# xmed-lab/NEURONS

Measured on AMD Instinct MI355X. Metric: denoising frames/sec, 16f x 256^2 clip, 50 DDIM steps, higher is better.
Workload: dtype bf16; 1 GPU; BASELINE config 2: 1 clip(s) per call, (1,4,16,32,32) latent, 50 DDIM steps, CFG 8.5 (batch 2), SparseCtrl + temporal U-Net per step, random-init weights; clips_per_gpu=5, ddim_steps=50, hip_graph=True, output_finite=True, attention=bf16

## Files before the change

neurons_amd/csrc/gemm_route.h:

```cpp
#pragma once
#include "common.h"
#include <cstdlib>
#include <initializer_list>

inline bool env_not_0(const char* name) {
  const char* v = getenv(name);
  return !(v && v[0] == '0');
}

inline int nr_plan_rows(const NrGemmParams& p) { return (p.plan_m > 0 && p.plan_m < p.M) ? p.plan_m : p.M; }

inline int nr_lds_opt_in(unsigned long long& mask, std::initializer_list<const void*> fns, size_t bytes) {
  int dev = 0;
  (void)hipGetDevice(&dev);
  const unsigned long long bit = 1ull << (dev & 63);
  if (mask & bit) return 0;
  for (const void* fn : fns)
    if (hipFuncSetAttribute(fn, hipFuncAttributeMaxDynamicSharedMemorySize, (int)bytes) != hipSuccess) return 2;
  mask |= bit;
  return 0;
}

enum NrGemmClass { NR_GEMM_SMALLM, NR_GEMM_LIN160, NR_GEMM_ROWPANEL, NR_GEMM_G8P, NR_GEMM_TILED, NR_GEMM_NCLASS };
inline const char* const nr_gemm_class_name[NR_GEMM_NCLASS] = {"smallm", "lin160", "rowpanel", "gemm8p", "tiled"};
enum NrWeightLayout { NR_W_ROWMAJOR, NR_W_TAP_INNER, NR_W_FRAGMAJOR, NR_W_LIN160, NR_W_LIN128Q, NR_W_FRAGMAJOR_E4M3 };

struct TiledPlan { int bm, bn, splitk, stages, waves, adma, lin; };
struct SmallmPlan { int nt, G, J, C; };
struct Lin160Plan { int form, big, J, cgmajor; };
struct RowPanelPlan { int nsplit; };
struct G8pPlan { int nt, phases; };

struct NrGemmRoute {
  int cls;
  int weight_layout;
  int m_fast;
  size_t ws_bytes;
  TiledPlan tiled;
  SmallmPlan smallm;
  Lin160Plan lin160;
  RowPanelPlan rowpanel;
  G8pPlan g8p;
};
```

neurons_amd/csrc/lin160.hip:

```cpp
#include "launchers.h"
#include "device_prims.h"
#include <cstdlib>

namespace {

NR_STAMP_BUF(lin160_stamp_buf, 512, 128);
#define L1_STAMP(slot) NR_STAMP_PUT(lin160_stamp_buf, slot)
#ifdef NR_STAMP_FINE
#define Q_STAMPW(slot) NR_STAMP_PUT_AT((threadIdx.x & 63) == 0 && (wave == 0 || wave == 4) && blockIdx.x < 256, lin160_stamp_buf, blockIdx.x + (wave ? 256 : 0), slot)
#else
#define Q_STAMPW(slot) do { } while (0)
#endif

constexpr int L1_BN = 160, L1_NT = 10;
constexpr int L1_W_STAGE = 24 * 1024;
constexpr int L1_NS = 3;

struct NrLin160Params {
  const bf16* x; int lda;
  const bf16* stream;
  const float* bias;
  const bf16* res; int ldr;
  bf16* out; int ldo;
  int M, N, K;
  const float* ln_c; float ln_eps;
  int norot;
};

template <int BM, int MODE = 0>
__global__ __launch_bounds__(512) void lin160_kernel(NrLin160Params p) {
  constexpr bool GLN = MODE == 1;
  static_assert(!GLN || BM == 128, "the GEGLU variant pairs the (value, gate) tiles inside one wave");
  constexpr int RT = BM / 16;
  constexpr int NTW = BM == 128 ? L1_NT : L1_NT / 2;
  constexpr int A_STAGE = BM * 128;
  constexpr int A_PW = BM == 128 ? 2 : 1;
  constexpr int STAGE = L1_W_STAGE + A_STAGE;
  constexpr int PPW = 3 + A_PW;
  extern __shared__ __attribute__((aligned(16))) unsigned char smem[];

  const int tid = threadIdx.x;
  const int lane = tid & 63;
  const int wave = __builtin_amdgcn_readfirstlane(tid >> 6);
  const int fr = lane & 15, fg = lane >> 4;
  const int rt = BM == 128 ? wave : (wave & 3);
  const int n0 = BM == 128 ? 0 : (wave >> 2) * NTW;

  L1_STAMP(0);
  const int NCB = p.N / L1_BN, S = p.K >> 6;
  const int nrg = p.M / BM;
  int rg, cb;
  if ((nrg & 7) == 0) { const int j = blockIdx.x >> 3; cb = j % NCB; rg = (j / NCB) * 8 + (int)(blockIdx.x & 7); }
  else { cb = (int)(blockIdx.x % NCB); rg = blockIdx.x / NCB; }
  const int r0 = rg * BM;
  const int rot = p.norot ? 0 : rg % S;

  const unsigned lds0 = nr_lds_addr(smem);
  const char* wsrc = reinterpret_cast<const char*>(p.stream) + (size_t)cb * ((size_t)S * L1_W_STAGE) + (size_t)(wave * 3) * 1024 + (size_t)lane * 16;
  const bf16* arow;
  {
    const int r = lane >> 2;
    arow = p.x + (size_t)(r0 + 16 * rt + r) * p.lda + (((lane & 3) ^ ((-(r >> 2)) & 3)) << 3);
  }
  auto issue_piece = [&](int s, int slot, int i) {
    const unsigned dst = lds0 + (unsigned)(slot * STAGE);
    int st = s + rot; if (st >= S) st -= S;
    if (i < 3) nr_glds16(wsrc + (size_t)st * L1_W_STAGE + (size_t)i * 1024, dst + (unsigned)((wave * 3 + i) * 1024));
    else {
      const int kk = BM == 128 ? i - 3 : (wave >> 2);
      nr_glds16(arow + 64 * st + 32 * kk, dst + (unsigned)(L1_W_STAGE + (kk * RT + rt) * 1024));
    }
  };
#pragma unroll
  for (int s = 0; s < L1_NS - 1; ++s)
#pragma unroll
    for (int i = 0; i < PPW; ++i) issue_piece(s, s, i);

  L1_STAMP(1);
  f32x4 acc[NTW];
#pragma unroll
  for (int n = 0; n < NTW; ++n) acc[n] = f32x4{0.f, 0.f, 0.f, 0.f};
  float s1 = 0.f, s2 = 0.f;
  const bf16x2 one2 = {(bf16)1.0f, (bf16)1.0f};
  const unsigned wl = (unsigned)(n0 * 1024 + lane * 16);
  const unsigned al = (unsigned)(L1_W_STAGE + rt * 1024 + fr * 64 + ((fg ^ ((-(fr >> 2)) & 3)) << 4));

  int slot = 0;
  for (int s = 0; s < S; ++s) {
    if (s + 1 < S) nr_wait_vmcnt<(L1_NS - 2) * PPW>(); else nr_wait_vmcnt<0>();
    if (s < 40) L1_STAMP(2 + 3 * s);
    __builtin_amdgcn_s_barrier();
    if (s < 40) L1_STAMP(3 + 3 * s);
    const int s_next = s + L1_NS - 1;
    const bool pf = s_next < S;
    int pslot = slot + L1_NS - 1; if (pslot >= L1_NS) pslot -= L1_NS;
    const unsigned char* base = smem + slot * STAGE;
#pragma unroll
    for (int kk = 0; kk < 2; ++kk) {
      const bf16x8 xa = *(const bf16x8*)(base + al + kk * (RT * 1024));
      if constexpr (GLN) {
#pragma unroll
        for (int e = 0; e < 4; ++e) {
          const bf16x2 pr = {xa[2 * e], xa[2 * e + 1]};
          s1 = __builtin_amdgcn_fdot2_f32_bf16(pr, one2, s1, false);
          s2 = __builtin_amdgcn_fdot2_f32_bf16(pr, pr, s2, false);
        }
      }
      bf16x8 w[NTW];
#pragma unroll
      for (int n = 0; n < NTW; ++n) w[n] = *(const bf16x8*)(base + (unsigned)((kk * L1_NT + n) * 1024) + wl);
      if (pf) {
        if (kk == 0) { issue_piece(s_next, pslot, 0); issue_piece(s_next, pslot, 1); }
        else { issue_piece(s_next, pslot, 2); issue_piece(s_next, pslot, 3); if (A_PW == 2) issue_piece(s_next, pslot, 4); }
      }
      __builtin_amdgcn_sched_barrier(0);
#pragma unroll
      for (int n = 0; n < NTW; ++n) acc[n] = __builtin_amdgcn_mfma_f32_16x16x32_bf16(w[n], xa, acc[n], 0, 0, 0);
      __builtin_amdgcn_sched_barrier(0);
    }
    if (s < 40) L1_STAMP(4 + 3 * s);
    slot = slot + 1 == L1_NS ? 0 : slot + 1;
  }
  L1_STAMP(125);

  if constexpr (GLN) {
    const float inv_k = 1.0f / (float)p.K;
    const float mu = nr_rows_sum(s1) * inv_k;
    const float rstd = rsqrtf(fmaxf(nr_rows_sum(s2) * inv_k - mu * mu, 0.f) + p.ln_eps);
    const int row = r0 + 16 * rt + fr;
    const int nb = cb * L1_BN + 4 * fg;
    bf16* orow = p.out + (size_t)row * p.ldo + cb * (L1_BN / 2) + 4 * fg;
#pragma unroll
    for (int i = 0; i < L1_NT / 2; ++i) {
      const int nv = nb + 32 * i, ng = nv + 16;
      const f32x4 cv = *(const f32x4*)(p.ln_c + nv), cg = *(const f32x4*)(p.ln_c + ng);
      const f32x4 bv = *(const f32x4*)(p.bias + nv), bg = *(const f32x4*)(p.bias + ng);
      bf16x4 o;
#pragma unroll
      for (int e = 0; e < 4; ++e) {
        const float v = (acc[2 * i][e] - mu * cv[e]) * rstd + bv[e];
        const float g = (acc[2 * i + 1][e] - mu * cg[e]) * rstd + bg[e];
        o[e] = (bf16)(v * gelu_erf_fast(g));
      }
      nr_store8(orow + 16 * i, o);
    }
    L1_STAMP(126);
    return;
  }
  const int row = r0 + 16 * rt + fr;
  const int cbase = cb * L1_BN + 16 * n0;
  bf16* orow = p.out + (size_t)row * p.ldo + cbase;
  const bf16* rrow = p.res ? p.res + (size_t)row * p.ldr + cbase : nullptr;
#pragma unroll
  for (int k = 0; k < NTW / 2; ++k) {
    f32x4 lo = acc[2 * k], hi = acc[2 * k + 1];
#pragma unroll
    for (int e = 0; e < 4; ++e) {
      auto sw = __builtin_amdgcn_permlane16_swap(__float_as_uint(lo[e]), __float_as_uint(hi[e]), false, false);
      lo[e] = __uint_as_float(sw[0]); hi[e] = __uint_as_float(sw[1]);
    }
    const int c = 16 * (2 * k + (fg & 1)) + 4 * (fg & 2);
    if (p.bias) { lo += *(const f32x4*)(p.bias + cbase + c); hi += *(const f32x4*)(p.bias + cbase + c + 4); }
    if (rrow) {
      const bf16x8 r = *(const bf16x8*)(rrow + c);
#pragma unroll
      for (int e = 0; e < 4; ++e) { lo[e] += (float)r[e]; hi[e] += (float)r[4 + e]; }
    }
    bf16x8 o;
#pragma unroll
    for (int e = 0; e < 4; ++e) { o[e] = (bf16)lo[e]; o[4 + e] = (bf16)hi[e]; }
    nr_store16(orow + c, o);
  }
  if constexpr (NTW % 2 == 1) {
    constexpr int n = NTW - 1;
    const int c = 16 * n + 4 * fg;
    f32x4 v = acc[n];
    if (p.bias) v += *(const f32x4*)(p.bias + cbase + c);
    if (rrow) {
      const bf16x4 r = *(const bf16x4*)(rrow + c);
#pragma unroll
      for (int e = 0; e < 4; ++e) v[e] += (float)r[e];
    }
    bf16x4 o;
#pragma unroll
    for (int e = 0; e < 4; ++e) o[e] = (bf16)v[e];
    nr_store8(orow + c, o);
  }
  L1_STAMP(126);
}

__global__ __launch_bounds__(256) void lin160_w_pack_kernel(const bf16* __restrict__ w, bf16* __restrict__ stream, int N, int K) {
  const int S = K >> 6, NCB = N / L1_BN, CH_STAGE = L1_W_STAGE / 16;
  const long long idx = (long long)blockIdx.x * 256 + threadIdx.x;
  if (idx >= (long long)NCB * S * CH_STAGE) return;
  const int cb = (int)(idx / ((long long)S * CH_STAGE));
  int c = (int)(idx - (long long)cb * S * CH_STAGE);
  const int st = c / CH_STAGE;
  c -= st * CH_STAGE;
  bf16x8 v = bf16x8_zero();
  if (c < 2 * L1_NT * 64) {
    const int kk = c / (L1_NT * 64), n = (c / 64) % L1_NT, lane = c & 63;
    v = *(const bf16x8*)(w + (size_t)(cb * L1_BN + 16 * n + (lane & 15)) * K + 64 * st + 32 * kk + 8 * (lane >> 4));
  }
  *(bf16x8*)(stream + (size_t)idx * 8) = v;
}


constexpr int Q_BN = 128, Q_NT = 8;
constexpr int Q_STAGE = 32 * 1024;
constexpr int Q_NS = 4;

struct NrLin128QParams {
  const bf16* x; int lda;
  const bf16* stream;
  const float* ln_c; const float* bias; float ln_eps;
  bf16* out; int ldo;
  int M, N, J, NCG;
  int norot;
  int cgmajor;
};

template <int KS, bool GEGLU, bool KSPLIT = false>
__global__ __launch_bounds__(512) void lin128q_kernel(NrLin128QParams p) {
  constexpr int K = 32 * KS;
  constexpr int KSL = KSPLIT ? KS / 2 : KS;
  constexpr int KPS = KSPLIT ? 8 : 4;
  constexpr int S = KS / KPS;
  constexpr int BN = KSPLIT ? 64 : Q_BN, NTB = BN / 16;
  constexpr int NS = KSPLIT ? 3 : Q_NS;
  constexpr int XCH = KSPLIT ? 32 * 1024 : 0;
  static_assert(KSL == 20 && S == 5, "20 k-steps per wave in 5 stages of 4");
  extern __shared__ __attribute__((aligned(16))) unsigned char smem[];
  const int tid = threadIdx.x;
  const int lane = tid & 63;
  const int wave = __builtin_amdgcn_readfirstlane(tid >> 6);
  const int fr = lane & 15, fg = lane >> 4;
  const int rp = wave & 3, ch = wave >> 2;
  L1_STAMP(0);
  const int J = p.J;
  int rg, cg;
  const int nrg = p.M >> 7;
  if (!p.cgmajor && (nrg & 7) == 0) { const int i = blockIdx.x >> 3; cg = i % p.NCG; rg = (i / p.NCG) * 8 + (int)(blockIdx.x & 7); }
  else { cg = (int)(blockIdx.x % p.NCG); rg = (int)(blockIdx.x / p.NCG); }
  const int row0 = rg * 128 + 32 * rp + fr;
  const int rot = p.norot ? 0 : rg % S;
  const int G = J * S;

  const unsigned lds0 = nr_lds_addr(smem);
  const char* wbase = reinterpret_cast<const char*>(p.stream) + (size_t)cg * J * ((size_t)S * Q_STAGE) + (size_t)(wave * 4) * 1024 + (size_t)lane * 16;
  auto issue_piece = [&](int g, int i) {
    const int gs = g < G ? g : G - 1;
    const int j = gs / S;
    int st = gs - j * S + rot; if (st >= S) st -= S;
    nr_glds16(wbase + ((size_t)j * S + st) * Q_STAGE + (size_t)i * 1024, lds0 + (unsigned)((g % NS) * Q_STAGE + (wave * 4 + i) * 1024));
  };
#pragma unroll
  for (int g = 0; g < NS - 1; ++g)
#pragma unroll
    for (int i = 0; i < 4; ++i) issue_piece(g, i);

  L1_STAMP(122);
  float* tab = reinterpret_cast<float*>(smem + NS * Q_STAGE + XCH);
  for (int i = tid; i < J * BN; i += 512) {
    tab[i] = p.ln_c[cg * J * BN + i];
    tab[J * BN + i] = p.bias[cg * J * BN + i];
  }

  L1_STAMP(123);
  bf16x8 xb[2][KSL];
#pragma unroll
  for (int rt = 0; rt < 2; ++rt) {
    const bf16* xr = p.x + (size_t)(row0 + 16 * rt) * p.lda + 8 * fg;
#pragma unroll
    for (int ks = 0; ks < KSL; ++ks) {
      int sq = (ks >> 2) + rot; if (sq >= S) sq -= S;
      const int kq = KPS * sq + (KSPLIT ? 4 * ch : 0) + (ks & 3);
      xb[rt][ks] = *(const bf16x8*)(xr + 32 * kq);
    }
  }
  L1_STAMP(124);
  float mu[2], rstd[2];
  {
    bf16x8 ones;
#pragma unroll
    for (int e = 0; e < 8; ++e) ones[e] = (bf16)1.0f;
    float sx[2], sq2[2];
#pragma unroll
    for (int rt = 0; rt < 2; ++rt) {
      f32x4 a1 = {0.f, 0.f, 0.f, 0.f}, a2 = {0.f, 0.f, 0.f, 0.f};
#pragma unroll
      for (int ks = 0; ks < KSL; ++ks) {
        a1 = __builtin_amdgcn_mfma_f32_16x16x32_bf16(ones, xb[rt][ks], a1, 0, 0, 0);
        a2 = __builtin_amdgcn_mfma_f32_16x16x32_bf16(xb[rt][ks], xb[rt][ks], a2, 0, 0, 0);
      }
      const int e_d = fr & 3;
      float d = e_d == 0 ? a2[0] : e_d == 1 ? a2[1] : e_d == 2 ? a2[2] : a2[3];
      d = (fg == (fr >> 2)) ? d : 0.f;
      sx[rt] = a1[0];
      sq2[rt] = nr_rows_sum(d);
    }
    if constexpr (KSPLIT) {
      float* xs = reinterpret_cast<float*>(smem + NS * Q_STAGE);
      if (fg == 0) {
#pragma unroll
        for (int rt = 0; rt < 2; ++rt) { xs[((wave * 2 + rt) * 2 + 0) * 16 + fr] = sx[rt]; xs[((wave * 2 + rt) * 2 + 1) * 16 + fr] = sq2[rt]; }
      }
      __builtin_amdgcn_s_barrier();
#pragma unroll
      for (int rt = 0; rt < 2; ++rt) { sx[rt] += xs[(((wave ^ 4) * 2 + rt) * 2 + 0) * 16 + fr]; sq2[rt] += xs[(((wave ^ 4) * 2 + rt) * 2 + 1) * 16 + fr]; }
    }
#pragma unroll
    for (int rt = 0; rt < 2; ++rt) {
      mu[rt] = sx[rt] * (1.0f / K);
      rstd[rt] = rsqrtf(fmaxf(sq2[rt] * (1.0f / K) - mu[rt] * mu[rt], 0.f) + p.ln_eps);
    }
  }
  L1_STAMP(127);
  nr_wait_vmcnt<0>();
  __builtin_amdgcn_s_barrier();
  L1_STAMP(1);

  const unsigned wl = (unsigned)((KSPLIT ? 16 * ch : 4 * ch) * 1024 + lane * 16);
  const unsigned oofs = (unsigned)row0 * (unsigned)p.ldo + (unsigned)((KSPLIT ? (GEGLU ? 16 * ch : 32 * ch) : (GEGLU ? 32 * ch : 64 * ch)) + 4 * fg);
  bf16x8 w[4];
#pragma unroll
  for (int n = 0; n < 4; ++n) w[n] = *(const bf16x8*)(smem + (unsigned)(n * 1024) + wl);
  f32x4 acc[2][4];
  auto epilogue = [&](int jb) {
    const int cb = cg * J + jb;
    constexpr int NF = KSPLIT ? 2 : 4;
    const float* tc = tab + jb * BN + 16 * (NF * ch) + 4 * fg;
    const float* tb = tc + J * BN;
    if constexpr (KSPLIT) {
      f32x4* ex = reinterpret_cast<f32x4*>(smem + NS * Q_STAGE);
#pragma unroll
      for (int rt = 0; rt < 2; ++rt)
#pragma unroll
        for (int nn = 0; nn < 2; ++nn) {
          f32x4 theirs;
#pragma unroll
          for (int e = 0; e < 4; ++e) theirs[e] = ch ? acc[rt][nn][e] : acc[rt][2 + nn][e];
          ex[((wave * 2 + rt) * 2 + nn) * 64 + lane] = theirs;
        }
      __builtin_amdgcn_s_barrier();
      const f32x4 c0 = *(const f32x4*)(tc), c1 = *(const f32x4*)(tc + 16), b0 = *(const f32x4*)(tb), b1 = *(const f32x4*)(tb + 16);
#pragma unroll
      for (int rt = 0; rt < 2; ++rt) {
        const f32x4 o0 = ex[(((wave ^ 4) * 2 + rt) * 2 + 0) * 64 + lane], o1 = ex[(((wave ^ 4) * 2 + rt) * 2 + 1) * 64 + lane];
        bf16x4 r0, r1;
#pragma unroll
        for (int e = 0; e < 4; ++e) {
          const float t0 = ((ch ? acc[rt][2][e] : acc[rt][0][e]) + o0[e] - mu[rt] * c0[e]) * rstd[rt] + b0[e];
          const float t1 = ((ch ? acc[rt][3][e] : acc[rt][1][e]) + o1[e] - mu[rt] * c1[e]) * rstd[rt] + b1[e];
          if constexpr (GEGLU) r0[e] = (bf16)(t0 * gelu_erf_fast(t1));
          else { r0[e] = (bf16)t0; r1[e] = (bf16)t1; }
        }
        bf16* orow = p.out + (oofs + (unsigned)(16 * rt) * (unsigned)p.ldo + (unsigned)(cb * (GEGLU ? BN / 2 : BN)));
        nr_store8(orow, r0);
        if constexpr (!GEGLU) nr_store8(orow + 16, r1);
      }
    } else if constexpr (GEGLU) {
#pragma unroll
      for (int i = 0; i < NF / 2; ++i) {
        const f32x4 cv = *(const f32x4*)(tc + 32 * i), cgv = *(const f32x4*)(tc + 32 * i + 16);
        const f32x4 bv = *(const f32x4*)(tb + 32 * i), bg = *(const f32x4*)(tb + 32 * i + 16);
#pragma unroll
        for (int rt = 0; rt < 2; ++rt) {
          bf16x4 o;
#pragma unroll
          for (int e = 0; e < 4; ++e) {
            const float v = (acc[rt][2 * i][e] - mu[rt] * cv[e]) * rstd[rt] + bv[e];
            const float gt = (acc[rt][2 * i + 1][e] - mu[rt] * cgv[e]) * rstd[rt] + bg[e];
            o[e] = (bf16)(v * gelu_erf_fast(gt));
          }
          nr_store8(p.out + (oofs + (unsigned)(16 * rt) * (unsigned)p.ldo + (unsigned)(cb * (BN / 2) + 16 * i)), o);
        }
      }
    } else {
#pragma unroll
      for (int n = 0; n < NF; ++n) {
        const f32x4 c4 = *(const f32x4*)(tc + 16 * n), b4 = *(const f32x4*)(tb + 16 * n);
#pragma unroll
        for (int rt = 0; rt < 2; ++rt) {
          bf16x4 o;
#pragma unroll
          for (int e = 0; e < 4; ++e) o[e] = (bf16)((acc[rt][n][e] - mu[rt] * c4[e]) * rstd[rt] + b4[e]);
          nr_store8(p.out + (oofs + (unsigned)(16 * rt) * (unsigned)p.ldo + (unsigned)(cb * BN + 16 * n)), o);
        }
      }
    }
  };
  const f32x4 zero4 = {0.f, 0.f, 0.f, 0.f};
  int g = 0, slot = 0;
  for (int j = 0; j < J; ++j) {
#pragma unroll
    for (int st = 0; st < S; ++st) {
      const int nslot = slot + 1 == NS ? 0 : slot + 1;
#pragma unroll
      for (int kk = 0; kk < 4; ++kk) {
        const unsigned char* nbase;
        if (kk < 3) nbase = smem + slot * Q_STAGE + (kk + 1) * (NTB * 1024);
        else {
          nr_wait_vmcnt<(NS - 2) * 4>();
          asm volatile("s_waitcnt lgkmcnt(0)" ::: "memory");
          if (g < 40) L1_STAMP(2 + 3 * g);
          __builtin_amdgcn_s_barrier();
          if (g < 40) L1_STAMP(3 + 3 * g);
          nbase = smem + nslot * Q_STAGE;
        }
        __builtin_amdgcn_sched_barrier(0);
        if (kk == 0) {
#pragma unroll
          for (int i = 0; i < 4; ++i) issue_piece(g + NS - 1, i);
        }
        __builtin_amdgcn_sched_barrier(0);
#pragma unroll
        for (int n = 0; n < 4; ++n) {
#pragma unroll
          for (int rt = 0; rt < 2; ++rt)
            acc[rt][n] = __builtin_amdgcn_mfma_f32_16x16x32_bf16(w[n], xb[rt][4 * st + kk], (st == 0 && kk == 0) ? zero4 : acc[rt][n], 0, 0, 0);
          __builtin_amdgcn_sched_barrier(0);
          w[n] = *(const bf16x8*)(nbase + (unsigned)(n * 1024) + wl);
          __builtin_amdgcn_sched_barrier(0);
        }
      }
      if (g < 40) L1_STAMP(4 + 3 * g);
      ++g;
      slot = nslot;
    }
    epilogue(j);
    if constexpr (KSPLIT) {
      __builtin_amdgcn_sched_barrier(0);
#pragma unroll
      for (int n = 0; n < 4; ++n) w[n] = *(const bf16x8*)(smem + slot * Q_STAGE + (unsigned)(n * 1024) + wl);
    }
  }
  L1_STAMP(125);
  nr_wait_vmcnt<0>();
  L1_STAMP(126);
}

__global__ __launch_bounds__(256) void lin128q_w_pack_kernel(const bf16* __restrict__ w, bf16* __restrict__ stream, int N, int K, int BN, int KPS) {
  const int S = K / (32 * KPS), CH_STAGE = Q_STAGE / 16, NTB = BN / 16;
  const long long idx = (long long)blockIdx.x * 256 + threadIdx.x;
  if (idx >= (long long)(N / BN) * S * CH_STAGE) return;
  const int cb = (int)(idx / ((long long)S * CH_STAGE));
  int c = (int)(idx - (long long)cb * S * CH_STAGE);
  const int st = c / CH_STAGE;
  c -= st * CH_STAGE;
  const int kk = c / (NTB * 64), n = (c / 64) % NTB, lane = c & 63;
  *(bf16x8*)(stream + (size_t)idx * 8) = *(const bf16x8*)(w + (size_t)(cb * BN + 16 * n + (lane & 15)) * K + 32 * (KPS * st + kk) + 8 * (lane >> 4));
}

}

#ifdef NR_STAMP
extern "C" int nr_lin160_stamp_read(void* dst, size_t bytes, int clear) { return nr_stamp_read_buf(lin160_stamp_buf, dst, bytes, clear); }
#endif

extern "C" size_t nr_lin160_stream_bytes(int N, int K) { return (N % L1_BN == 0 && K % 64 == 0) ? (size_t)(N / L1_BN) * (K / 64) * L1_W_STAGE : 0; }

extern "C" int nr_lin160_panel_rule(int Mp, int N, int K) {
  static const bool off = !env_not_0("NR_LIN160") || !env_not_0("NR_LIN160_PANEL");
  static const bool off1280 = !env_not_0("NR_LIN160_PANEL_K1280");
  static const int maxm = getenv("NR_LIN160_PANEL_MAXM") ? atoi(getenv("NR_LIN160_PANEL_MAXM")) : (1 << 30);
  if (off || Mp < 2048 || Mp > maxm || N < 3 * K) return 0;
  if (K == 640) return Mp >= 4096 && N % Q_BN == 0;
  if (K == 1280) return !off1280 && N % 64 == 0;
  return 0;
}
extern "C" size_t nr_lin128q_stream_bytes(int N, int K) {
  if (K == 640) return N % Q_BN == 0 ? (size_t)N * K * sizeof(bf16) : 0;
  if (K == 1280) return N % 64 == 0 ? (size_t)N * K * sizeof(bf16) : 0;
  return 0;
}
extern "C" int nr_launch_lin128q_w_pack(const bf16* w, int N, int K, bf16* stream, hipStream_t s) {
  const long long total = (long long)(nr_lin128q_stream_bytes(N, K) / 16);
  if (!total) return 1;
  hipLaunchKernelGGL(lin128q_w_pack_kernel, dim3((unsigned)((total + 255) / 256)), dim3(256), 0, s, w, stream, N, K, K == 1280 ? 64 : Q_BN, K == 1280 ? 8 : 4);
  return 0;
}

extern "C" bool lin160_plan(const NrGemmParams& p, Lin160Plan* pl) {
  static const bool off = !env_not_0("NR_LIN160");
  const int Mp = nr_plan_rows(p);
  *pl = Lin160Plan{0, 0, 0, 0};
  const bool ln_wide = p.ln_c && p.bias && p.ksize == 1 && p.stride == 1 && !p.ups && !p.a1 && !p.c1 && !p.rowvec && !p.act && !p.out_f32 && !p.res &&
                       p.out_scale == 1.0f && p.K == p.c0 && p.M % 128 == 0 && p.lda0 % 8 == 0 && p.ldo % 4 == 0;
  if (ln_wide && nr_lin160_panel_rule(Mp, p.N, p.K) &&
      (long long)p.M * p.ldo < (1ll << 31)) {
    const bool ksplit = p.K == 1280;
    const int bn = ksplit ? 64 : Q_BN, ncq = p.N / bn, S = 5, nrg = p.M / 128, ns = ksplit ? 3 : Q_NS;
    static const int j_force = getenv("NR_LIN160_PANEL_J") ? atoi(getenv("NR_LIN160_PANEL_J")) : 0;
    int J = 0; long long best = 0;
    for (int c = 1; c <= 16 && c <= ncq; ++c) {
      if (ncq % c != 0 || c * S < ns - 1) continue;
      const long long wgs = (long long)nrg * (ncq / c), cost = ((wgs + 255) / 256) * (c * S + 6);
      if (!J || cost <= best) { J = c; best = cost; }
    }
    if (j_force > 0 && ncq % j_force == 0 && j_force <= 16) J = j_force;
    pl->form = 4; pl->J = J;
    if (J) {
      static const int cg_force = getenv("NR_LIN160_PANEL_CGMAJOR") ? atoi(getenv("NR_LIN160_PANEL_CGMAJOR")) : -1;
      const int NCG = ncq / J;
      const double wb = 2.0 * p.N * (double)p.K, xb = 2.0 * p.M * (double)p.K;
      const bool can = NCG % 8 == 0 || 8 % NCG == 0;
      const double by_rg = 8.0 * wb + xb;
      const double by_cg = (NCG % 8 == 0 ? 1.0 : 8.0 / NCG) * wb + (NCG % 8 == 0 ? 8.0 : (double)NCG) * xb;
      pl->cgmajor = (can && by_cg < by_rg) ? 1 : 0;
      if (cg_force >= 0) pl->cgmajor = cg_force && can;
    }
    return true;
  }
  static const bool gln_on = env_not_0("NR_LIN160_GEGLU");
  if (!off && gln_on && ln_wide && p.geglu && p.K == 1280 && p.N % L1_BN == 0 && p.N >= 8192 && Mp <= 1024 && (long long)(Mp / 128) * (p.N / L1_BN) >= 192) {
    pl->form = 2;
    return true;
  }
  if (off || p.ksize != 1 || p.stride != 1 || p.ups || p.a1 || p.c1 || p.geglu || p.ln_c || p.rowvec || p.act || p.out_f32 || p.tap_inner) return false;
  if (p.out_scale != 1.0f || p.K != p.c0 || (p.K != 640 && p.K != 1280) || p.N % L1_BN != 0 || p.N > 1280) return false;
  if (p.M % 64 != 0 || Mp < 2048) return false;
  if (p.lda0 % 8 != 0 || p.ldo % 8 != 0 || (p.res && p.ldr % 8 != 0)) return false;
  if (Mp > 8192) return false;
  pl->form = 1;
  pl->big = p.M % 128 == 0 && (long long)(Mp / 128) * (p.N / L1_BN) >= 256;
  return true;
}

extern "C" int nr_launch_lin160_w_pack(const bf16* w, int N, int K, bf16* stream, hipStream_t s) {
  const long long total = (long long)(nr_lin160_stream_bytes(N, K) / 16);
  if (!total) return 1;
  hipLaunchKernelGGL(lin160_w_pack_kernel, dim3((unsigned)((total + 255) / 256)), dim3(256), 0, s, w, stream, N, K);
  return 0;
}

extern "C" int nr_launch_lin160(const NrGemmParams* pp, const Lin160Plan* pl, const bf16* stream, hipStream_t s) {
  const NrGemmParams& g = *pp;
  if (!stream) return 1;
  if (pl->form == 4) {
    const bool ksplit = g.K == 1280;
    if (!g.ln_c || !g.bias || (g.K != 640 && !ksplit) || g.M % 128 != 0 || (long long)g.M * g.ldo >= (1ll << 31)) return 1;
    const int bn = ksplit ? 64 : Q_BN, ncq = g.N / bn, nrg = g.M / 128, ns = ksplit ? 3 : Q_NS, J = pl->J;
    if (g.N % bn != 0 || J < 1 || J > 16 || ncq % J != 0) return 1;
    NrLin128QParams q;
    q.x = g.a0; q.lda = g.lda0; q.stream = stream; q.ln_c = g.ln_c; q.bias = g.bias; q.ln_eps = g.ln_eps; q.out = g.out; q.ldo = g.ldo; q.M = g.M; q.N = g.N; q.norot = g.plan_m > 0 ? 1 : 0;
    q.J = J; q.NCG = ncq / J; q.cgmajor = pl->cgmajor;
    const size_t shm_max = (size_t)Q_NS * Q_STAGE + 2 * 16 * Q_BN * sizeof(float);
    const size_t shm = (size_t)ns * Q_STAGE + (ksplit ? 32 * 1024 : 0) + (size_t)2 * J * bn * sizeof(float);
    typedef void (*kern_t)(NrLin128QParams);
    static const kern_t ks[4] = {lin128q_kernel<20, true>, lin128q_kernel<20, false>, lin128q_kernel<40, true, true>, lin128q_kernel<40, false, true>};
    static unsigned long long done[4] = {};
    const int ki = (ksplit ? 2 : 0) + (g.geglu ? 0 : 1);
    if (const int rc = nr_lds_opt_in(done[ki], {(const void*)ks[ki]}, shm_max)) return rc;
    hipLaunchKernelGGL(ks[ki], dim3((unsigned)(nrg * q.NCG)), dim3(512), shm, s, q);
    return 0;
  }
  if (g.M % 64 != 0 || g.N % L1_BN != 0 || g.K % 64 != 0 || g.K / 64 < L1_NS) return 1;
  NrLin160Params p;
  p.x = g.a0; p.lda = g.lda0; p.stream = stream; p.bias = g.bias; p.res = g.res; p.ldr = g.ldr; p.out = g.out; p.ldo = g.ldo; p.M = g.M; p.N = g.N; p.K = g.K; p.norot = g.plan_m > 0 ? 1 : 0;
  const int ncb = g.N / L1_BN;
  p.ln_c = g.ln_c; p.ln_eps = g.ln_eps;
  const bool gln = pl->form == 2, big = gln || pl->big;
  if (gln != (g.geglu != 0) || (gln && (!g.ln_c || !g.bias)) || (big && g.M % 128 != 0)) return 1;
  typedef void (*kern_t)(NrLin160Params);
  static const kern_t ks[3] = {lin160_kernel<128, 1>, lin160_kernel<128, 0>, lin160_kernel<64, 0>};
  const int ki = gln ? 0 : (big ? 1 : 2), rows = big ? 128 : 64;
  const size_t shm = (size_t)L1_NS * (L1_W_STAGE + rows * 128);
  static unsigned long long done[3] = {};
  if (const int rc = nr_lds_opt_in(done[ki], {(const void*)ks[ki]}, shm)) return rc;
  hipLaunchKernelGGL(ks[ki], dim3((unsigned)((g.M / rows) * ncb)), dim3(512), shm, s, p);
  return 0;
}
```

Measured before the change: 20.03 frames/s.

## Add lin160 wave variants: 32-row waves, residual prefetch, and skipped pad-weight loads

Adds templated variants of the lin160 GEMM kernel. In the W32 form each wave covers two 16-row tiles across half the N columns, so every weight fragment read from LDS feeds two MFMAs. The RESPF form loads the residual tile into registers before the K loop, taking that latency out of the epilogue. The NOPAD form skips the weight pieces that only fill the padded region of each stage and adjusts the per-wave vmcnt waits to match. All three are on by default through environment flags, which raises register pressure and brings in more kernel instances and dispatch logic.

```diff
diff --git a/neurons_amd/csrc/gemm_route.h b/neurons_amd/csrc/gemm_route.h
--- a/neurons_amd/csrc/gemm_route.h
+++ b/neurons_amd/csrc/gemm_route.h
@@ -27,7 +27,7 @@
 
 struct TiledPlan { int bm, bn, splitk, stages, waves, adma, lin; };
 struct SmallmPlan { int nt, G, J, C; };
-struct Lin160Plan { int form, big, J, cgmajor; };
+struct Lin160Plan { int form, big; union { int J; int waves; }; int cgmajor; };
 struct RowPanelPlan { int nsplit; };
 struct G8pPlan { int nt, phases; };
 
diff --git a/neurons_amd/csrc/lin160.hip b/neurons_amd/csrc/lin160.hip
--- a/neurons_amd/csrc/lin160.hip
+++ b/neurons_amd/csrc/lin160.hip
@@ -27,12 +27,66 @@
   int norot;
 };
 
+#define L1_EPILOGUE_TILE(rr)                                                                                                                                                       \
+{                                                                                                                                                     \
+  const int row = r0 + 16 * (rt + (rr)) + fr;                                                                                                         \
+  const int cbase = cb * L1_BN + 16 * n0;                                                                                                             \
+  bf16* orow = p.out + (size_t)row * p.ldo + cbase;                                                                                                   \
+  const bf16* rrow = p.res ? p.res + (size_t)row * p.ldr + cbase : nullptr;                                                        \
+  _Pragma("unroll")                                                                                                                                   \
+  for (int k = 0; k < NTW / 2; ++k) {                                                                                                                 \
+    f32x4 lo = acc[rr][2 * k], hi = acc[rr][2 * k + 1];                                                                                               \
+    _Pragma("unroll")                                                                                                                                 \
+    for (int e = 0; e < 4; ++e) {                                                                                                                     \
+      auto sw = __builtin_amdgcn_permlane16_swap(__float_as_uint(lo[e]), __float_as_uint(hi[e]), false, false);                                       \
+      lo[e] = __uint_as_float(sw[0]); hi[e] = __uint_as_float(sw[1]);                                                                                 \
+    }                                                                                                                                                 \
+    const int c = 16 * (2 * k + (fg & 1)) + 4 * (fg & 2);                                                                                             \
+    if (p.bias) { lo += *(const f32x4*)(p.bias + cbase + c); hi += *(const f32x4*)(p.bias + cbase + c + 4); }                                         \
+    if constexpr (RESPF) {                                                                                                                            \
+      _Pragma("unroll")                                                                                                                               \
+      for (int e = 0; e < 4; ++e) { lo[e] += (float)rpair[rr][k][e]; hi[e] += (float)rpair[rr][k][4 + e]; }                                           \
+    } else if (rrow) {                                                                                                                                \
+      const bf16x8 r = *(const bf16x8*)(rrow + c);                                                                                                    \
+      _Pragma("unroll")                                                                                                                               \
+      for (int e = 0; e < 4; ++e) { lo[e] += (float)r[e]; hi[e] += (float)r[4 + e]; }                                                                 \
+    }                                                                                                                                                 \
+    bf16x8 o;                                                                                                                                         \
+    _Pragma("unroll")                                                                                                                                 \
+    for (int e = 0; e < 4; ++e) { o[e] = (bf16)lo[e]; o[4 + e] = (bf16)hi[e]; }                                                                       \
+    nr_store16(orow + c, o);                                                                                                                          \
+  }                                                                                                                                                   \
+  if constexpr (NTW % 2 == 1) {                                                                                                                       \
+    constexpr int n = NTW - 1;                                                                                                                        \
+    const int c = 16 * n + 4 * fg;                                                                                                                    \
+    f32x4 v = acc[rr][n];                                                                                                                             \
+    if (p.bias) v += *(const f32x4*)(p.bias + cbase + c);                                                                                             \
+    if constexpr (RESPF) {                                                                                                                            \
+      _Pragma("unroll")                                                                                                                               \
+      for (int e = 0; e < 4; ++e) v[e] += (float)rodd[rr][e];                                                                                         \
+    } else if (rrow) {                                                                                                                                \
+      const bf16x4 r = *(const bf16x4*)(rrow + c);                                                                                                    \
+      _Pragma("unroll")                                                                                                                               \
+      for (int e = 0; e < 4; ++e) v[e] += (float)r[e];                                                                                                \
+    }                                                                                                                                                 \
+    bf16x4 o;                                                                                                                                         \
+    _Pragma("unroll")                                                                                                                                 \
+    for (int e = 0; e < 4; ++e) o[e] = (bf16)v[e];                                                                                                    \
+    nr_store8(orow + c, o);                                                                                                                           \
+  }\
+}
+
+constexpr int L1_W32 = 1, L1_RESPF = 2, L1_NOPAD = 4;
 template <int BM, int MODE = 0>
 __global__ __launch_bounds__(512) void lin160_kernel(NrLin160Params p) {
   constexpr bool GLN = MODE == 1;
+  constexpr bool W32 = MODE >= 2 && ((MODE >> 1) & L1_W32) != 0, RESPF = MODE >= 2 && ((MODE >> 1) & L1_RESPF) != 0, NOPAD = MODE >= 2 && ((MODE >> 1) & L1_NOPAD) != 0;
+  static_assert(MODE >= 0 && MODE <= 2 * (L1_W32 | L1_RESPF | L1_NOPAD) && (MODE < 2 || MODE % 2 == 0), "0, 1 or twice a wave form");
   static_assert(!GLN || BM == 128, "the GEGLU variant pairs the (value, gate) tiles inside one wave");
+  static_assert(!W32 || BM == 128, "32-row waves: the 128-row tile");
   constexpr int RT = BM / 16;
-  constexpr int NTW = BM == 128 ? L1_NT : L1_NT / 2;
+  constexpr int NRT = W32 ? 2 : 1;
+  constexpr int NTW = (BM == 128 && !W32) ? L1_NT : L1_NT / 2;
   constexpr int A_STAGE = BM * 128;
   constexpr int A_PW = BM == 128 ? 2 : 1;
   constexpr int STAGE = L1_W_STAGE + A_STAGE;
@@ -43,8 +97,8 @@
   const int lane = tid & 63;
   const int wave = __builtin_amdgcn_readfirstlane(tid >> 6);
   const int fr = lane & 15, fg = lane >> 4;
-  const int rt = BM == 128 ? wave : (wave & 3);
-  const int n0 = BM == 128 ? 0 : (wave >> 2) * NTW;
+  const int rt = W32 ? 2 * (wave & 3) : BM == 128 ? wave : (wave & 3);
+  const int n0 = (BM == 128 && !W32) ? 0 : (wave >> 2) * NTW;
 
   L1_STAMP(0);
   const int NCB = p.N / L1_BN, S = p.K >> 6;
@@ -60,26 +114,41 @@
   const bf16* arow;
   {
     const int r = lane >> 2;
-    arow = p.x + (size_t)(r0 + 16 * rt + r) * p.lda + (((lane & 3) ^ ((-(r >> 2)) & 3)) << 3);
+    arow = p.x + (size_t)(r0 + 16 * (W32 ? wave : rt) + r) * p.lda + (((lane & 3) ^ ((-(r >> 2)) & 3)) << 3);
   }
   auto issue_piece = [&](int s, int slot, int i) {
     const unsigned dst = lds0 + (unsigned)(slot * STAGE);
     int st = s + rot; if (st >= S) st -= S;
-    if (i < 3) nr_glds16(wsrc + (size_t)st * L1_W_STAGE + (size_t)i * 1024, dst + (unsigned)((wave * 3 + i) * 1024));
-    else {
+    if (i < 3) {
+      if (!NOPAD || wave * 3 + i < 2 * L1_NT) nr_glds16(wsrc + (size_t)st * L1_W_STAGE + (size_t)i * 1024, dst + (unsigned)((wave * 3 + i) * 1024));
+    } else {
       const int kk = BM == 128 ? i - 3 : (wave >> 2);
-      nr_glds16(arow + 64 * st + 32 * kk, dst + (unsigned)(L1_W_STAGE + (kk * RT + rt) * 1024));
+      nr_glds16(arow + 64 * st + 32 * kk, dst + (unsigned)(L1_W_STAGE + (kk * RT + (W32 ? wave : rt)) * 1024));
     }
   };
+  bf16x8 rpair[NRT][NTW / 2 > 0 ? NTW / 2 : 1];
+  bf16x4 rodd[NRT];
+  if constexpr (RESPF) {
+#pragma unroll
+    for (int r = 0; r < NRT; ++r) {
+      const bf16* rrow = p.res + (size_t)(r0 + 16 * (rt + r) + fr) * p.ldr + cb * L1_BN + 16 * n0;
+#pragma unroll
+      for (int k = 0; k < NTW / 2; ++k) rpair[r][k] = *(const bf16x8*)(rrow + 16 * (2 * k + (fg & 1)) + 4 * (fg & 2));
+      if constexpr (NTW % 2 == 1) rodd[r] = *(const bf16x4*)(rrow + 16 * (NTW - 1) + 4 * fg);
+    }
+    __builtin_amdgcn_sched_barrier(0);
+  }
 #pragma unroll
   for (int s = 0; s < L1_NS - 1; ++s)
 #pragma unroll
     for (int i = 0; i < PPW; ++i) issue_piece(s, s, i);
 
   L1_STAMP(1);
-  f32x4 acc[NTW];
-#pragma unroll
-  for (int n = 0; n < NTW; ++n) acc[n] = f32x4{0.f, 0.f, 0.f, 0.f};
+  f32x4 acc[NRT][NTW];
+#pragma unroll
+  for (int r = 0; r < NRT; ++r)
+#pragma unroll
+    for (int n = 0; n < NTW; ++n) acc[r][n] = f32x4{0.f, 0.f, 0.f, 0.f};
   float s1 = 0.f, s2 = 0.f;
   const bf16x2 one2 = {(bf16)1.0f, (bf16)1.0f};
   const unsigned wl = (unsigned)(n0 * 1024 + lane * 16);
@@ -87,6 +156,12 @@
 
   int slot = 0;
   for (int s = 0; s < S; ++s) {
+    if constexpr (NOPAD) {
+      if (s + 1 == S) nr_wait_vmcnt<0>();
+      else if (wave < 6) nr_wait_vmcnt<(L1_NS - 2) * PPW>();
+      else if (wave == 6) nr_wait_vmcnt<(L1_NS - 2) * (PPW - 1)>();
+      else nr_wait_vmcnt<(L1_NS - 2) * (PPW - 3)>();
+    } else
     if (s + 1 < S) nr_wait_vmcnt<(L1_NS - 2) * PPW>(); else nr_wait_vmcnt<0>();
     if (s < 40) L1_STAMP(2 + 3 * s);
     __builtin_amdgcn_s_barrier();
@@ -97,11 +172,13 @@
     const unsigned char* base = smem + slot * STAGE;
 #pragma unroll
     for (int kk = 0; kk < 2; ++kk) {
-      const bf16x8 xa = *(const bf16x8*)(base + al + kk * (RT * 1024));
+      bf16x8 xa[NRT];
+#pragma unroll
+      for (int r = 0; r < NRT; ++r) xa[r] = *(const bf16x8*)(base + al + (kk * RT + r) * 1024);
       if constexpr (GLN) {
 #pragma unroll
         for (int e = 0; e < 4; ++e) {
-          const bf16x2 pr = {xa[2 * e], xa[2 * e + 1]};
+          const bf16x2 pr = {xa[0][2 * e], xa[0][2 * e + 1]};
           s1 = __builtin_amdgcn_fdot2_f32_bf16(pr, one2, s1, false);
           s2 = __builtin_amdgcn_fdot2_f32_bf16(pr, pr, s2, false);
         }
@@ -115,7 +192,9 @@
       }
       __builtin_amdgcn_sched_barrier(0);
 #pragma unroll
-      for (int n = 0; n < NTW; ++n) acc[n] = __builtin_amdgcn_mfma_f32_16x16x32_bf16(w[n], xa, acc[n], 0, 0, 0);
+      for (int n = 0; n < NTW; ++n)
+#pragma unroll
+        for (int r = 0; r < NRT; ++r) acc[r][n] = __builtin_amdgcn_mfma_f32_16x16x32_bf16(w[n], xa[r], acc[r][n], 0, 0, 0);
       __builtin_amdgcn_sched_barrier(0);
     }
     if (s < 40) L1_STAMP(4 + 3 * s);
@@ -138,8 +217,8 @@
       bf16x4 o;
 #pragma unroll
       for (int e = 0; e < 4; ++e) {
-        const float v = (acc[2 * i][e] - mu * cv[e]) * rstd + bv[e];
-        const float g = (acc[2 * i + 1][e] - mu * cg[e]) * rstd + bg[e];
+        const float v = (acc[0][2 * i][e] - mu * cv[e]) * rstd + bv[e];
+        const float g = (acc[0][2 * i + 1][e] - mu * cg[e]) * rstd + bg[e];
         o[e] = (bf16)(v * gelu_erf_fast(g));
       }
       nr_store8(orow + 16 * i, o);
@@ -147,47 +226,11 @@
     L1_STAMP(126);
     return;
   }
-  const int row = r0 + 16 * rt + fr;
-  const int cbase = cb * L1_BN + 16 * n0;
-  bf16* orow = p.out + (size_t)row * p.ldo + cbase;
-  const bf16* rrow = p.res ? p.res + (size_t)row * p.ldr + cbase : nullptr;
-#pragma unroll
-  for (int k = 0; k < NTW / 2; ++k) {
-    f32x4 lo = acc[2 * k], hi = acc[2 * k + 1];
-#pragma unroll
-    for (int e = 0; e < 4; ++e) {
-      auto sw = __builtin_amdgcn_permlane16_swap(__float_as_uint(lo[e]), __float_as_uint(hi[e]), false, false);
-      lo[e] = __uint_as_float(sw[0]); hi[e] = __uint_as_float(sw[1]);
-    }
-    const int c = 16 * (2 * k + (fg & 1)) + 4 * (fg & 2);
-    if (p.bias) { lo += *(const f32x4*)(p.bias + cbase + c); hi += *(const f32x4*)(p.bias + cbase + c + 4); }
-    if (rrow) {
-      const bf16x8 r = *(const bf16x8*)(rrow + c);
-#pragma unroll
-      for (int e = 0; e < 4; ++e) { lo[e] += (float)r[e]; hi[e] += (float)r[4 + e]; }
-    }
-    bf16x8 o;
-#pragma unroll
-    for (int e = 0; e < 4; ++e) { o[e] = (bf16)lo[e]; o[4 + e] = (bf16)hi[e]; }
-    nr_store16(orow + c, o);
-  }
-  if constexpr (NTW % 2 == 1) {
-    constexpr int n = NTW - 1;
-    const int c = 16 * n + 4 * fg;
-    f32x4 v = acc[n];
-    if (p.bias) v += *(const f32x4*)(p.bias + cbase + c);
-    if (rrow) {
-      const bf16x4 r = *(const bf16x4*)(rrow + c);
-#pragma unroll
-      for (int e = 0; e < 4; ++e) v[e] += (float)r[e];
-    }
-    bf16x4 o;
-#pragma unroll
-    for (int e = 0; e < 4; ++e) o[e] = (bf16)v[e];
-    nr_store8(orow + c, o);
-  }
+  L1_EPILOGUE_TILE(0)
+  if constexpr (NRT == 2) L1_EPILOGUE_TILE(1)
   L1_STAMP(126);
 }
+#undef L1_EPILOGUE_TILE
 
 __global__ __launch_bounds__(256) void lin160_w_pack_kernel(const bf16* __restrict__ w, bf16* __restrict__ stream, int N, int K) {
   const int S = K >> 6, NCB = N / L1_BN, CH_STAGE = L1_W_STAGE / 16;
@@ -484,7 +527,7 @@
 extern "C" bool lin160_plan(const NrGemmParams& p, Lin160Plan* pl) {
   static const bool off = !env_not_0("NR_LIN160");
   const int Mp = nr_plan_rows(p);
-  *pl = Lin160Plan{0, 0, 0, 0};
+  *pl = Lin160Plan{};
   const bool ln_wide = p.ln_c && p.bias && p.ksize == 1 && p.stride == 1 && !p.ups && !p.a1 && !p.c1 && !p.rowvec && !p.act && !p.out_f32 && !p.res &&
                        p.out_scale == 1.0f && p.K == p.c0 && p.M % 128 == 0 && p.lda0 % 8 == 0 && p.ldo % 4 == 0;
   if (ln_wide && nr_lin160_panel_rule(Mp, p.N, p.K) &&
@@ -524,6 +567,8 @@
   if (Mp > 8192) return false;
   pl->form = 1;
   pl->big = p.M % 128 == 0 && (long long)(Mp / 128) * (p.N / L1_BN) >= 256;
+  static const bool w32 = env_not_0("NR_LIN160_W32"), respf = env_not_0("NR_LIN160_RESPF"), nopad = env_not_0("NR_LIN160_NOPAD");
+  pl->waves = (w32 && pl->big ? L1_W32 : 0) | (respf && p.res && (pl->big || nopad) ? L1_RESPF : 0) | (nopad ? L1_NOPAD : 0);
   return true;
 }
 
@@ -563,10 +608,16 @@
   const bool gln = pl->form == 2, big = gln || pl->big;
   if (gln != (g.geglu != 0) || (gln && (!g.ln_c || !g.bias)) || (big && g.M % 128 != 0)) return 1;
   typedef void (*kern_t)(NrLin160Params);
-  static const kern_t ks[3] = {lin160_kernel<128, 1>, lin160_kernel<128, 0>, lin160_kernel<64, 0>};
-  const int ki = gln ? 0 : (big ? 1 : 2), rows = big ? 128 : 64;
+  static const kern_t ks[3 + 8 + 4] = {lin160_kernel<128, 1>, lin160_kernel<128, 0>, lin160_kernel<64, 0>,
+                                       lin160_kernel<128, 0>, lin160_kernel<128, 2>, lin160_kernel<128, 4>, lin160_kernel<128, 6>, lin160_kernel<128, 8>, lin160_kernel<128, 10>,
+                                       lin160_kernel<128, 12>, lin160_kernel<128, 14>, lin160_kernel<64, 0>, lin160_kernel<64, 4>, lin160_kernel<64, 8>, lin160_kernel<64, 12>};
+  int wf = gln ? 0 : pl->waves;
+  if (wf & ~(L1_W32 | L1_RESPF | L1_NOPAD)) return 1;
+  if (!big) wf &= ~L1_W32;
+  if (!g.res) wf &= ~L1_RESPF;
+  const int ki = gln ? 0 : (wf == 0 ? (big ? 1 : 2) : (big ? 3 + wf : 11 + (wf >> 1))), rows = big ? 128 : 64;
   const size_t shm = (size_t)L1_NS * (L1_W_STAGE + rows * 128);
-  static unsigned long long done[3] = {};
+  static unsigned long long done[3 + 8 + 4] = {};
   if (const int rc = nr_lds_opt_in(done[ki], {(const void*)ks[ki]}, shm)) return rc;
   hipLaunchKernelGGL(ks[ki], dim3((unsigned)((g.M / rows) * ncb)), dim3(512), shm, s, p);
   return 0;
```

Measured after the change: 20.15 frames/s, median of 6. Within noise of the previous version (+0.6%).
